# stanfordnlp/mac-network

Hardware: AMD Instinct MI355X
Metric: questions/sec fwd+bwd (B=64,d=512,p=12,KB=14x14x1024) at 1/2/4/8 MI355X (higher is better)
Workload: dtype f32 (3xfp16-split emulation); 1 GPU

## Files before the change

include/macx.h:

```cpp
#ifndef MACX_H
#define MACX_H

#include <stddef.h>
#include <stdint.h>

#ifdef __cplusplus
extern "C" {
#endif

#define MACX_ABI_VERSION 5

enum {
  MACX_OK = 0,
  MACX_EINVAL = -1,
  MACX_EUNSUPPORTED = -2,
  MACX_EREJECTED = -3,
  MACX_ESMALL = -4,
  MACX_EWAIT = -5
};

enum { MACX_ACT_NON = 0, MACX_ACT_TANH = 1, MACX_ACT_SIGMOID = 2, MACX_ACT_ELU = 3, MACX_ACT_RELU = 4 };
enum { MACX_INIT_PRM = 0, MACX_INIT_ZERO = 1, MACX_INIT_Q = 2 };
enum { MACX_WRITE_MEM = 0, MACX_WRITE_INFO = 1, MACX_WRITE_SUM = 2, MACX_WRITE_BOTH = 3 };

typedef struct macx_opts {
  int32_t abi_version;
  int32_t init_ctrl, init_mem;
  int32_t control_input_unshared;
  int32_t control_input_act;
  int32_t control_feed_prev;
  int32_t control_feed_prev_att;
  int32_t control_feed_inputs;
  int32_t control_cont_act;
  int32_t read_mem_act;
  int32_t read_ctrl_act;
  int32_t write_inputs;
  int32_t write_self_att;
  int32_t write_self_att_cont;
  int32_t write_mem_act;
  int32_t write_gate;
  int32_t write_gate_shared;
  float   write_gate_bias;
  int32_t memory_variational_dropout;
  int32_t gemm_family;
  int32_t tune[16];
} macx_opts;
#define MACX_TUNE(v) ((v) + 1)
enum {
  MACX_TUNE_NATIVE_WAVES = 0,
  MACX_TUNE_PHASE_MASK = 1,
  MACX_TUNE_ROW_TILES = 2,
  MACX_TUNE_CHAIN = 4,
  MACX_TUNE_SB_DEFER = 5,
  MACX_TUNE_CHAIN_KV = 7,
  MACX_TUNE_SB_WIDE = 8,
  MACX_TUNE_WGRAD_PIPE = 10,
  MACX_TUNE_SB_CONT = 13,
  MACX_TUNE_DKB_UNI = 14,
  MACX_TUNE_PRE_FILL = 3,
  MACX_TUNE_DKB_FILL = 15
};

typedef struct macx_shapes {
  int32_t B;
  int32_t S;
  int32_t N;
  int32_t d;
  int32_t p;
  int32_t b0;
  int32_t d_logical;
} macx_shapes;

typedef struct macx_dropout {
  float keep_memory, keep_read, keep_write;
  uint32_t seed;
  const uint32_t* mask_word;
} macx_dropout;

typedef struct macx_params {
  const float* initMem;
  const float* initCtrl;
  const float* qInput_W;
  const float* qInput_b;
  const float* qInputU_W;
  const float* qInputU_b;
  const float* ctrlLogits_w;
  const float* ctrlLogits_b;
  const float* contControl_W;
  const float* contControl_b;
  const float* contControl2_W;
  const float* contControl2_b;
  const float* projX_W;
  const float* projX_b;
  const float* projY_W;
  const float* projY_b;
  const float* memKbProj_W;
  const float* memKbProj_b;
  const float* memKbProj2_W;
  const float* memKbProj2_b;
  const float* kbLogits_w;
  const float* kbLogits_b;
  const float* newMemory_W;
  const float* newMemory_b;
  const float* selfCtrl_W;
  const float* selfCtrl_b;
  const float* selfLogits_w;
  const float* selfLogits_b;
  const float* gate_W;
  const float* gate_b;
} macx_params;

typedef struct macx_param_grads {
  float* initMem; float* initCtrl;
  float* qInput_W; float* qInput_b; float* qInputU_W; float* qInputU_b;
  float* ctrlLogits_w; float* ctrlLogits_b;
  float* contControl_W; float* contControl_b; float* contControl2_W; float* contControl2_b;
  float* projX_W; float* projX_b; float* projY_W; float* projY_b;
  float* memKbProj_W; float* memKbProj_b; float* memKbProj2_W; float* memKbProj2_b;
  float* kbLogits_w; float* kbLogits_b;
  float* newMemory_W; float* newMemory_b;
  float* selfCtrl_W; float* selfCtrl_b; float* selfLogits_w; float* selfLogits_b;
  float* gate_W; float* gate_b;
} macx_param_grads;

typedef struct macx_inputs {
  const float* vecQuestions;
  const float* words;
  const int32_t* questionLengths;
  const float* knowledgeBase;
} macx_inputs;

typedef struct macx_input_grads {
  float* vecQuestions;
  float* words;
  float* knowledgeBase;
} macx_input_grads;

enum {
  MACX_SEG_CONTROLS = 0,
// ... 207 lines not shown
```

mac-network_amd/_lib.py:

```python
import ctypes as C
import os

from . import build as _build

ABI_VERSION = 5

MACX_OK, MACX_EINVAL, MACX_EUNSUPPORTED, MACX_EREJECTED, MACX_ESMALL, MACX_EWAIT = 0, -1, -2, -3, -4, -5
HANDOFF_BITS = {1: "a chain tile gave up waiting for its step's y", 2: "a filler workgroup gave up waiting for the previous step's write unit"}
STATUS_WORDS = 16
ACT = {"NON": 0, "TANH": 1, "SIGMOID": 2, "ELU": 3, "RELU": 4}
INIT = {"PRM": 0, "ZERO": 1, "Q": 2}
WRITE_INPUTS = {"MEM": 0, "INFO": 1, "SUM": 2, "BOTH": 3}
SEG = {"controls": 0, "memories": 1, "infos": 2, "att_question": 3, "att_kb": 4, "att_self": 5, "att_gate": 6,
       "status": 7}


class MacxOpts(C.Structure):
    _fields_ = [(n, C.c_int32) for n in (
        "abi_version", "init_ctrl", "init_mem", "control_input_unshared", "control_input_act", "control_feed_prev",
        "control_feed_prev_att", "control_feed_inputs", "control_cont_act", "read_mem_act", "read_ctrl_act",
        "write_inputs", "write_self_att", "write_self_att_cont", "write_mem_act", "write_gate", "write_gate_shared")]
    _fields_ += [("write_gate_bias", C.c_float), ("memory_variational_dropout", C.c_int32), ("gemm_family", C.c_int32),
                 ("tune", C.c_int32 * 16)]


TUNE = {"native_waves": 0, "phase_mask": 1, "row_tiles": 2, "pre_fill": 3, "chain": 4, "sb_defer": 5, "chain_kv": 7, "sb_wide": 8,
        "wgrad_pipe": 10, "sb_cont": 13, "dkb_uni": 14, "dkb_fill": 15}


def set_tune(opts, key, value):
    k = TUNE[key] if isinstance(key, str) else int(key)
    if k not in TUNE.values():
        raise KeyError("no tuning key %r (have %s)" % (key, sorted(TUNE)))
    opts.tune[k] = 0 if value is None else int(value) + 1


class MacxShapes(C.Structure):
    _fields_ = [(n, C.c_int32) for n in ("B", "S", "N", "d", "p", "b0", "d_logical")]


class MacxDropout(C.Structure):
    _fields_ = [("keep_memory", C.c_float), ("keep_read", C.c_float), ("keep_write", C.c_float), ("seed", C.c_uint32),
                ("mask_word", C.c_void_p)]


PARAM_FIELDS = (
    "initMem", "initCtrl", "qInput_W", "qInput_b", "qInputU_W", "qInputU_b", "ctrlLogits_w", "ctrlLogits_b",
    "contControl_W", "contControl_b", "contControl2_W", "contControl2_b", "projX_W", "projX_b", "projY_W", "projY_b",
    "memKbProj_W", "memKbProj_b", "memKbProj2_W", "memKbProj2_b", "kbLogits_w", "kbLogits_b", "newMemory_W",
    "newMemory_b", "selfCtrl_W", "selfCtrl_b", "selfLogits_w", "selfLogits_b", "gate_W", "gate_b")


class MacxParams(C.Structure):
    _fields_ = [(n, C.c_void_p) for n in PARAM_FIELDS]


class MacxParamGrads(C.Structure):
    _fields_ = [(n, C.c_void_p) for n in PARAM_FIELDS]


class MacxOutShapes(C.Structure):
    _fields_ = [(n, C.c_int32) for n in ("B", "d", "hidden", "answers", "b0")]


OUT_FIELDS = ("outQuestion_W", "outQuestion_b", "fc0_W", "fc0_b", "fc1_W", "fc1_b")


class MacxOutParams(C.Structure):
    _fields_ = [(n, C.c_void_p) for n in OUT_FIELDS]


class MacxOutGrads(C.Structure):
    _fields_ = [(n, C.c_void_p) for n in OUT_FIELDS]


class MacxStemShapes(C.Structure):
    _fields_ = [(n, C.c_int32) for n in ("B", "H", "W", "Cin", "Cmid", "Cout", "b0")]


STEM_FIELDS = ("kernel0", "bias0", "kernel1", "bias1")


class MacxStemParams(C.Structure):
    _fields_ = [(n, C.c_void_p) for n in STEM_FIELDS]


class MacxStemGrads(C.Structure):
    _fields_ = [(n, C.c_void_p) for n in STEM_FIELDS]


class MacxConvShapes(C.Structure):
    _fields_ = [(n, C.c_int32) for n in ("B", "H", "W", "Cin", "Cout", "k", "stride")]


class MacxEncShapes(C.Structure):
    _fields_ = [(n, C.c_int32) for n in ("B", "S", "V", "E", "h", "b0")]


ENC_FIELDS = ("emb", "fw_kernel", "fw_bias", "bw_kernel", "bw_bias")


class MacxEncParams(C.Structure):
    _fields_ = [(n, C.c_void_p) for n in ENC_FIELDS]


class MacxEncGrads(C.Structure):
    _fields_ = [(n, C.c_void_p) for n in ENC_FIELDS]


# ... 191 lines not shown
```

mac-network_amd/csrc/macx_api.hip:

```cpp
#include <hip/hip_runtime.h>
#include <math.h>
#include <stdlib.h>
#include <string.h>

#include "../../include/macx.h"
#include "macx_common.hip.h"
#include "macx_gemm.hip.h"
#include "macx_gemm6.hip.h"
#include "macx_gemm_tn.hip.h"
#include "macx_wgrad6.hip.h"
#include "macx_gemm3h.hip.h"
#include "macx_h2.hip.h"
#include "macx_gemm_h2.hip.h"
#include "macx_chain_api.hip.h"
#include "macx_wgrad_h2.hip.h"
#include "macx_small.hip.h"
#include "macx_ops.hip.h"
#include "macx_conv.hip.h"

using namespace macx;

#define CK(expr)                         \
  do {                                   \
    hipError_t _e = (expr);              \
// ... 1642 lines not shown
}

int CellBwd::initial_state_bwd() {
  if (o->init_mem == MACX_INIT_PRM) CK(rs.add(DM, B, d, d, GP->initMem, st));
  else if (o->init_mem == MACX_INIT_Q && o->init_ctrl == MACX_INIT_Q) CK(axpy(DM, Bd, GI->vecQuestions, st));
  if (o->init_ctrl == MACX_INIT_PRM) CK(rs.add(DC, B, d, d, GP->initCtrl, st));
  return MACX_OK;
}

int CellBwd::read_linear_wgrads() {
  CKI(wb.add(saved + L.md, d, ws + W.DY, d, p * B, d, d, GP->projY_W, st));
  CK(rs.add(ws + W.DY, p * B, d, d, GP->projY_b, st));
  return MACX_OK;
}

int CellBwd::write_linear_wgrads() {
  const int rows = p * B;
  CKI(wb.add(memories(), d, dwlin_all, d, rows, d, d, GP->newMemory_W, st));
  CKI(wb.add(saved + L.seg[MACX_SEG_INFOS], d, dwlin_all, d, rows, d, d, GP->newMemory_W + dd, st));
  if (o->write_self_att)
    CKI(wb.add(saved + L.self_smry, d, dwlin_all, d, rows, d, d, GP->newMemory_W + 2 * dd, st));
  CK(rs.add(dwlin_all, rows, d, d, GP->newMemory_b, st));
  return MACX_OK;
}

int CellBwd::read_weight_contractions() {
  int ns_w = (int)W.ns_big;
  if (h2) {
    int* ecom = reinterpret_cast<int*>(ws + W.ecom);
    constexpr int ES = EMIN_NB * 8;
    {
      EminList el;
      memset(&el, 0, sizeof(el));
      el.R = B * N; el.C = d; el.part = ecom;
      el.base[0] = reinterpret_cast<const char*>(saved + L.H1); el.stride[0] = L.act_stride * sizeof(float); el.nt[0] = p;
      el.base[1] = reinterpret_cast<const char*>(ws + W.dI2); el.stride[1] = W.act_floats * sizeof(float); el.nt[1] = p;
      el.base[2] = reinterpret_cast<const char*>(saved + L.KBd); el.stride[2] = L.act_stride * sizeof(float); el.nt[2] = rdrop ? p : 1;
      el.base[3] = reinterpret_cast<const char*>(ws + W.dX); el.stride[3] = W.act_floats * sizeof(float); el.nt[3] = p;
      CK(emin_list(el, 4, st));
    }
    TnH2P t;
    memset(&t, 0, sizeof(t));
    ns_w = (wgrad_pipe_mode() >= 3 && wgrad_h2_kw(d) == 2 && wgrad_h2_jw(d) == 2 && W.ns_big >= 2) ? (int)W.ns_big / 2 : (int)W.ns_big;
    t.M = p * B * N; t.Kd = d; t.Jd = d; t.nsplit = ns_w; t.rows_per_split = rows_per_split(t.M, t.nsplit);
    t.R = B * N;
    t.A = reinterpret_cast<const char*>(saved + L.H1); t.a_stride = L.act_stride * sizeof(float); t.a_mod = 0;
    t.G = reinterpret_cast<const char*>(ws + W.dI2); t.g_stride = W.act_floats * sizeof(float);
    t.ecomA = ecom; t.ecomG = ecom + ES; t.ecom_nb = EMIN_NB;
    t.ftab = reinterpret_cast<uint16_t*>(ws + W.wg_ftab);
    t.dbg = kb_gemm_dbg();
    t.part = ws + W.slab_w2;
    const TnH2P t_w2 = t;
    t.A = reinterpret_cast<const char*>(saved + L.KBd);
    t.a_mod = rdrop ? 0 : B * N;
    t.G = reinterpret_cast<const char*>(ws + W.dX);
    t.ecomA = ecom + 2 * ES; t.ecomG = ecom + 3 * ES;
    t.part = ws + W.slab_wx;
    t.ftab = reinterpret_cast<uint16_t*>(ws + W.wg_ftab2);
    CK(wgrad_h2_launch_pair(t_w2, t, st));
  } else {
    TnP t;
    memset(&t, 0, sizeof(t));
    t.M = p * B * N; t.Kd = d; t.Jd = d; t.nsplit = (int)W.ns_big; t.rows_per_split = rows_per_split(t.M, t.nsplit);
    t.A = saved + L.H1; t.lda = d; t.a_mod = t.M; t.G = ws + W.dI2; t.ldg = d;
    t.part = ws + W.slab_w2;
    CK(wgrad_any(t, st));
    if (rdrop) { t.A = saved + L.KBd; t.a_mod = t.M; }
    else { t.A = in->knowledgeBase; t.a_mod = B * N; }
    t.G = ws + W.dX;
    t.part = ws + W.slab_wx;
    CK(wgrad_any(t, st));
  }
  if (h2 && W.sb_deferred) {
    SbH2P q;
    memset(&q, 0, sizeof(q));
    q.B = B; q.N = N; q.d = d; q.qpg = sb_qpg(B, N);
    q.X = h2_view(saved + L.X, B * N, d); q.dI1 = h2_view(ws + W.dI1, B * N, d);
    q.y = saved + L.y; q.W1a = P->memKbProj_W;
    q.dW1a_part = ws + W.slab_w1a; q.dW1b_part = ws + W.slab_w1b; q.dy_part = nullptr;
    q.nsteps = p;
    q.x_step = L.act_stride * sizeof(float); q.g_step = W.dI1_stride * sizeof(float); q.y_step = Bd;
    q.dbg = kb_gemm_dbg();
    q.qpg = W.sb_qpg;
    CK(W.sb_wide ? sb_h2w_launch(q, st) : sb_h2_launch(q, st));
  }
  const int nslab1 = (int)((h2 && W.sb_deferred ? 1 : p) * W.ngroup);
  SlabList sl;
  sl.d[0] = SlabDesc{ws + W.slab_w2, ns_w, dd / 4, GP->memKbProj2_W, 0};
  sl.d[1] = SlabDesc{ws + W.slab_wx, ns_w, dd / 4, GP->projX_W, 0};
  sl.d[2] = SlabDesc{ws + W.slab_w1a, nslab1, dd / 4, GP->memKbProj_W, 0};
  sl.d[3] = SlabDesc{ws + W.slab_w1b, nslab1, dd / 4, GP->memKbProj_W + dd, 0};
  CK(slab_reduce_list_launch(sl, 4, dd, st));
  CK(rs.add(ws + W.db2_part, p * (int)W.dwk_rows, d, d, GP->memKbProj2_b, st));
  CK(rs.add(ws + W.db1_part, p * (int)W.db_rows, d, d, GP->memKbProj_b, st));
  CK(rs.add(ws + W.dbx_part, p * (int)W.db_rows, d, d, GP->projX_b, st));
  CK(rs.add(ws + W.dwk_part, p * (int)W.dwk_rows, d, d, GP->kbLogits_w, st));
  CK(rs.add(ws + W.dbk_part, p * B, 1, 1, GP->kbLogits_b, st));
  CK(rs.run(st));
  return MACX_OK;
}
}

int macx_cell_backward_phase(const macx_opts* o, const macx_shapes* s, const macx_dropout* dp, const macx_params* P,
                             const macx_inputs* in, const float* saved, size_t saved_floats, float* ws, size_t ws_floats,
                             const float* d_memory, const float* d_control, const macx_param_grads* GP,
                             const macx_input_grads* GI, int phase, void* stream) {
  ModeScope ms(o);
  if (phase < 0 || phase > 2) return MACX_EINVAL;
  CKI(check_impl(o, s));
  if (!dp || !P || !in || !saved || !ws || !GP || !GI) return MACX_EINVAL;
  if (!GI->knowledgeBase || !GI->words || !GI->vecQuestions) return MACX_EINVAL;
  CellBwd r(o, s, dp, P, in, saved, ws, GP, GI, stream);
  CKI(r.check_bwd_buffers(saved_floats, ws_floats, phase));
  if (phase != 2) {
    CKI(r.init_state_grads(d_memory, d_control));
    if (o->control_feed_prev) {
      CK(dev_zero(GI->words, (size_t)r.B * s->S * r.d * sizeof(float), r.st));
      CK(dev_zero(ws + r.W.dwc_part, r.Bd * sizeof(float), r.st));
      CK(dev_zero(ws + r.W.dccx, (size_t)(r.p + 1) * r.Bd * sizeof(float), r.st));
      r.dc_in_loop = true;
    }
    r.plan_dkb_fill();
    for (int i = r.p - 1; i >= 0; --i) {
      CKI(r.write_unit_bwd(i));
      CKI(r.read_unit_bwd(i));
      CKI(r.dy_linear_bwd(i, true));
      if (o->control_feed_prev) CKI(r.control_step_bwd(i));
    }
    CKI(r.read_dc_reduce_all());
    CKI(r.control_bwd_tail());
    CKI(r.gate_wgrads());
    CKI(r.control_inputs_bwd());
    CKI(r.initial_state_bwd());
    CKI(r.read_linear_wgrads());
    CKI(r.write_linear_wgrads());
    CKI(r.wb.run(r.st));
  }
  CK(r.rs.run(r.st));
  return phase == 1 ? MACX_OK : r.read_weight_contractions();
}

int macx_cell_backward(const macx_opts* o, const macx_shapes* s, const macx_dropout* dp, const macx_params* P,
                       const macx_inputs* in, const float* saved, size_t saved_floats, float* ws, size_t ws_floats,
                       const float* d_memory, const float* d_control, const macx_param_grads* GP,
                       const macx_input_grads* GI, void* stream) {
  return macx_cell_backward_phase(o, s, dp, P, in, saved, saved_floats, ws, ws_floats, d_memory, d_control, GP, GI, 0, stream);
}

namespace {
int unit_check(const macx_opts* o, const macx_shapes* s, bool write) {
  CKI(check_impl(o, s));
  if (s->p != 1) return MACX_EINVAL;
  if (write && o->write_self_att) return MACX_EUNSUPPORTED;
  return MACX_OK;
}
}

size_t macx_workspace_bytes(const macx_opts* o, const macx_shapes* s, int for_backward) {
  return macx_ws_floats(o, s, for_backward) * sizeof(float);
}

int macx_read_fwd(const macx_opts* o, const macx_shapes* s, const macx_dropout* dp, const macx_params* P,
                  const float* knowledgeBase, const float* memory, const float* control, float* saved, size_t saved_floats,
                  float* info, float* att, void* stream) {
  ModeScope ms(o);
  CKI(unit_check(o, s, false));
// ... 1137 lines not shown
```

mac-network_amd/csrc/macx_wgrad_h2.hip.h:

```cpp
#pragma once
#include "macx_gemm_tn.hip.h"
#include "macx_h2.hip.h"

namespace macx {

__device__ __forceinline__ float sum16_h2(float v) {
  v += __shfl_xor(v, 1, 64);
  v += __shfl_xor(v, 2, 64);
  v += __shfl_xor(v, 4, 64);
  v += __shfl_xor(v, 8, 64);
  return v;
}
__device__ __forceinline__ uint32_t pk_mul_f16(uint32_t a, uint32_t b) {
  return __builtin_bit_cast(uint32_t, __builtin_bit_cast(f16x2_t, a) * __builtin_bit_cast(f16x2_t, b));
}
__device__ __forceinline__ uint32_t pk_pow2_f16(int k) {
  const float f = k < -30 ? 0.f : h2_pow2(k);
  return pk_f16(f, f);
}

struct ReadAttBwdH2P {
  int B, N, d;
  const float* att;
  const float* da;
// ... 412 lines not shown
          wh_mfma<NR, NC>(af, gf[0], acc);
        }
        if (p.dbg & 2048) wait_vmcnt<0>(); else wait_vmcnt_n(my_n);
        __syncthreads();
      }
      wait_vmcnt<0>();
    }
  } else
  if (nchunk > 0) {
    const int my_n = (NI + (wave == 0 ? 1 : 0)) * (RING - 2);
#pragma unroll
    for (int s = 0; s < RING - 1; ++s) issue(s);
    wait_vmcnt_n(my_n);
    __syncthreads();
#pragma unroll 1
    for (int s = 0; s < nchunk; ++s) {
      if (!(p.dbg & 2048)) issue(s + RING - 1);
      if (!(p.dbg & 1024)) wh_compute<NR, NC>(tiles_a(s % RING), APL, tiles_g(s % RING), GPL, factors(s % RING), lane, acc);
      wait_vmcnt_n(my_n);
      __syncthreads();
    }
    wait_vmcnt<0>();
  }

  __syncthreads();

  const float sc = h2_unscale(h2_emin_final(p.ecomA, p.ecom_nb, tk * KW + aq), h2_emin_final(p.ecomG, p.ecom_nb, tj * JW + gq));
  float* out = p.part + (size_t)split * p.Kd * p.Jd + (size_t)(tk * KT + wr * 16 * NR) * p.Jd + tj * JT + wc * 32 * JW;
  float* tw = reinterpret_cast<float*>(lds) + wave * (32 * wh_slab_ldw<NC>());
#pragma unroll
  for (int tp = 0; tp < NR; tp += 2) wh_store_slab<2>(acc, tp, sc, tw, out, p.Jd, lane);
}

inline int wgrad_h2_jw(int Jd) { return (Jd % 256 == 0) ? 2 : 1; }
inline int wgrad_h2_kw(int Kd) { return (Kd % 256 == 0) ? 2 : 1; }
inline int wgrad_h2_tiles(int Kd, int Jd) { return (Kd / (wgrad_h2_kw(Kd) * T_TILE)) * (Jd / (wgrad_h2_jw(Jd) * T_TILE)); }

inline hipError_t wgrad_h2_factors_launch(const TnH2P& a, const TnH2P& b, int ny, hipStream_t st) {
  if (a.rows_per_split % 32 != 0 || !a.ftab || !b.ftab) return hipErrorInvalidValue;
  const size_t mpad = wgrad_h2_mpad((size_t)a.M);
  hipLaunchKernelGGL(wgrad_h2_factors_kernel, dim3((unsigned)((mpad + 255) / 256), ny), dim3(256), 0, st, a, b);
  return hipGetLastError();
}
template <int KW, int JW, int PIPE = 0>
inline hipError_t wgrad_h2_launch_t(const TnH2P& a, const TnH2P& b, int ny, hipStream_t st) {
  auto kern = wgrad_h2_kernel<KW, JW, PIPE>;
  constexpr size_t lds = (size_t)wh_ring<KW, JW>() * wh_stage_bytes<KW, JW>();
  hipError_t e = lds_attr_once(reinterpret_cast<const void*>(kern), lds);
  if (e != hipSuccess) return e;
  hipLaunchKernelGGL(kern, dim3(wgrad_h2_tiles(a.Kd, a.Jd) * a.nsplit, ny), dim3(512), lds, st, a, b);
  return hipGetLastError();
}
inline hipError_t wgrad_h2_launch(const TnH2P& p, hipStream_t st) {
  hipError_t e = wgrad_h2_factors_launch(p, p, 1, st);
  if (e != hipSuccess) return e;
  const int kw = wgrad_h2_kw(p.Kd), jw = wgrad_h2_jw(p.Jd);
  if (kw == 2 && jw == 2) return wgrad_pipe_mode() ? wgrad_h2_launch_t<2, 2, 1>(p, p, 1, st) : wgrad_h2_launch_t<2, 2, 0>(p, p, 1, st);
  if (kw == 2) return wgrad_h2_launch_t<2, 1>(p, p, 1, st);
  return jw == 2 ? wgrad_h2_launch_t<1, 2>(p, p, 1, st) : wgrad_h2_launch_t<1, 1>(p, p, 1, st);
}
inline hipError_t wgrad_h2_launch_pair(const TnH2P& a, const TnH2P& b, hipStream_t st) {
  const bool same = a.M == b.M && a.Kd == b.Kd && a.Jd == b.Jd && a.nsplit == b.nsplit && a.rows_per_split == b.rows_per_split && a.R == b.R;
  if (!(same && wgrad_pipe_mode() >= 2 && wgrad_h2_kw(a.Kd) == 2 && wgrad_h2_jw(a.Jd) == 2 && a.ftab != b.ftab && a.part != b.part)) {
    hipError_t e = wgrad_h2_launch(a, st);
    return e != hipSuccess ? e : wgrad_h2_launch(b, st);
  }
  hipError_t e = wgrad_h2_factors_launch(a, b, 2, st);
  return e != hipSuccess ? e : wgrad_h2_launch_t<2, 2, 1>(a, b, 2, st);
}

struct SbH2P {
  int B, N, d;
  int qpg;
  H2View X;
  H2View dI1;
  const float* y;
  const float* W1a;
  float* dW1a_part;
  float* dW1b_part;
  float* dy_part;
  int nsteps;
  size_t x_step, g_step, y_step;
  int dbg;
};

constexpr int SBH_STAGE = 4 * WH_APL;
constexpr int SBH_CW = 8;
constexpr int SBH_MAXROWS = 4096;
constexpr int SBH_RING = 4;
constexpr int SBH_MAXQ = 32;

template <bool DY>
__global__ __launch_bounds__(512) void sb_h2_kernel(SbH2P p) {
  extern __shared__ __attribute__((aligned(16))) float smem[];
  char* lds = reinterpret_cast<char*>(smem);
  uint16_t* ftab = reinterpret_cast<uint16_t*>(lds + SBH_RING * SBH_STAGE);
  float* ytab = reinterpret_cast<float*>(lds + SBH_RING * SBH_STAGE + SBH_MAXROWS * 2);
  float* sctab = ytab + SBH_MAXQ * T_TILE;
  int* qmn = reinterpret_cast<int*>(sctab + SBH_MAXQ);

  const int nt = p.d / T_TILE;
  const int ntile = nt * nt;
  const int nblk = gridDim.x;
  int v = blockIdx.x;
  if ((nblk & 7) == 0) v = (blockIdx.x & 7) * (nblk >> 3) + (blockIdx.x >> 3);
  const int group = v / ntile;
  const int tile = v % ntile;
  const int tk = tile / nt, tj = tile % nt;

  const int tid = threadIdx.x, lane = tid & 63;
  const int wave = __builtin_amdgcn_readfirstlane(tid >> 6);
  const int wr = wave >> 2, wc = wave & 3;

  const int nchunk = (p.N + 31) >> 5;
  const int b_begin = group * p.qpg;
  const int b_end = min(p.B, b_begin + p.qpg);
  const int nq = b_end - b_begin;
  const int total = nq * nchunk;
  const size_t Rp = p.X.Rp();
  const size_t xpb = p.X.plane_bytes(), gpb = p.dI1.plane_bytes();
  const int xcb = p.X.cb(), gcb = p.dI1.cb();
  H2View vX = p.X, vG = p.dI1;
  const float* yS = p.y;
  const int rows_q = nchunk * 32;

  const WhSlot sl = wh_slot(lane);
  auto issue = [&](int s_raw) __attribute__((always_inline)) {
    const int s = min(s_raw, total - 1);
    const int qi = s / nchunk, ch = s - qi * nchunk;
    const int n = sl.row(ch * 32, p.N);
    const size_t row = (size_t)(b_begin + qi) * p.N + n;
    char* st = lds + (s_raw % SBH_RING) * SBH_STAGE;
#pragma unroll
    for (int j = 0; j < 4; ++j) {
      const int u = wave * 4 + j;
      const int im = u >> 3, ct = u & 7;
      const char* src = (im < 2 ? vX.base + (im & 1) * xpb + ((size_t)(tk * 16 + 2 * ct + sl.kg) * Rp + row) * 16
                                : vG.base + (im & 1) * gpb + ((size_t)(tj * 16 + 2 * ct + sl.kg) * Rp + row) * 16);
      dma16b(src, st + im * WH_APL + ct * 1024);
    }
  };
  auto tables = [&]() __attribute__((always_inline)) {
  if (tid < 2 * SBH_MAXQ) qmn[tid] = 127;
  __syncthreads();
  for (int i0 = 0; i0 < nq * rows_q; i0 += 512) {
    const int i = i0 + tid;
    const int qi = i / rows_q, n = i - qi * rows_q;
    int ex = 127, eg = 127;
    if (i < nq * rows_q && n < p.N) {
      const size_t row = (size_t)(b_begin + qi) * p.N + n;
      ex = (int)vX.exps()[row * xcb + tk];
      eg = (int)vG.exps()[row * gcb + tj];
    }
    const int q_lo = min(i0 + (tid & ~63), nq * rows_q - 1) / rows_q, q_hi = min(i0 + (tid | 63), nq * rows_q - 1) / rows_q;
    for (int q = q_lo; q <= q_hi; ++q) {
      int mx = qi == q ? ex : 127, mg = qi == q ? eg : 127;
#pragma unroll
      for (int o = 32; o > 0; o >>= 1) { mx = min(mx, __shfl_xor(mx, o, 64)); mg = min(mg, __shfl_xor(mg, o, 64)); }
      if (lane == 0) { atomicMin(qmn + q, mx); atomicMin(qmn + SBH_MAXQ + q, mg); }
    }
  }
  __syncthreads();
  for (int i = tid; i < nq * rows_q; i += 512) {
    const int qi = i / rows_q, n = i - qi * rows_q;
    const int b = b_begin + qi;
    uint16_t f = 0;
// ... 38 lines not shown
  auto consume = [&](int b) __attribute__((always_inline)) {
    const float sc = sctab[b - b_begin];
    f32x4 y4[4];
#pragma unroll
    for (int t = 0; t < 4; ++t) y4[t] = *reinterpret_cast<const f32x4*>(ytab + (b - b_begin) * T_TILE + wr * 64 + t * 16 + (lane >> 4) * 4);
#pragma unroll
    for (int t = 0; t < 4; ++t)
#pragma unroll
      for (int e = 0; e < 4; ++e) {
        const int k = tk * T_TILE + wr * 64 + t * 16 + (lane >> 4) * 4 + e;
        const float yk = y4[t][e];
        float dyp = 0.f;
#pragma unroll
        for (int c = 0; c < 2; ++c) {
          const float sv = accS[t][c][e] * sc;
          accB[t][c][e] += sv;
          accA[t][c][e] = fmaf(yk, sv, accA[t][c][e]);
          if (DY) dyp = fmaf(w1[t][e][c], sv, dyp);
          accS[t][c][e] = 0.f;
        }
        if (DY) {
          dyp = sum16_h2(dyp);
          if ((lane & 15) == 0) p.dy_part[((size_t)(tj * 4 + wc) * p.B + b) * p.d + k] = dyp;
        }
      }
  };

#pragma unroll 1
  for (int step = 0; step < p.nsteps; ++step) {
  vX.base = p.X.base + (size_t)step * p.x_step; vG.base = p.dI1.base + (size_t)step * p.g_step;
  yS = p.y + (size_t)step * p.y_step;
  if (total > 0) {
    issue(0);
    issue(1);
    issue(2);
  }
  tables();
  if (total > 0) {
    wait_vmcnt<8>();
    __syncthreads();
    int qi = 0, qch = 0;
#pragma unroll 1
    for (int s = 0; s < total; ++s) {
      if (!(p.dbg & 2048)) issue(s + 3);
      if (!(p.dbg & 1024)) compute(s % SBH_RING, qi, qch);
      wait_vmcnt<8>();
      if (++qch == nchunk) {
        if (!(p.dbg & 512)) consume(b_begin + qi);
        qch = 0; ++qi;
      }
      __syncthreads();
    }
    wait_vmcnt<0>();
  }
  __syncthreads();
  }

  float* oa = p.dW1a_part + (size_t)group * p.d * p.d;
  float* ob = p.dW1b_part + (size_t)group * p.d * p.d;
  constexpr int LDW = 36;
  float* tw = reinterpret_cast<float*>(lds) + wave * (64 * LDW);
#pragma unroll
  for (int which = 0; which < 2; ++which) {
#pragma unroll
    for (int t = 0; t < 4; ++t)
#pragma unroll
      for (int c = 0; c < 2; ++c)
#pragma unroll
        for (int e = 0; e < 4; ++e)
          tw[(t * 16 + (lane >> 4) * 4 + e) * LDW + c * 16 + (lane & 15)] = which ? accB[t][c][e] : accA[t][c][e];
    float* o = (which ? ob : oa) + (size_t)(tk * T_TILE + wr * 64) * p.d + tj * T_TILE + wc * 32;
#pragma unroll
    for (int i = 0; i < 8; ++i) {
      const int r = i * 8 + (lane >> 3), c4 = (lane & 7) * 4;
      *reinterpret_cast<f32x4*>(o + (size_t)r * p.d + c4) = *reinterpret_cast<const f32x4*>(tw + r * LDW + c4);
    }
  }
}

constexpr int SBW_STAGE = 2 * WH_APL + 4 * WH_APL;
constexpr int SBW_RING = 3;
constexpr int SBW_MAXQ = 4;
constexpr int SBW_MAXROWS = 1024;

constexpr int SBW_TABLES = SBW_MAXROWS * 2 + SBW_MAXQ * T_TILE * 4 + 4 * SBW_MAXQ * 4;
template <bool CONT>
__global__ __launch_bounds__(512) void sb_h2w_kernel(SbH2P p) {
  extern __shared__ __attribute__((aligned(16))) float smem[];
  char* lds = reinterpret_cast<char*>(smem);
  char* tab0 = lds + SBW_RING * SBW_STAGE;
  uint16_t* ftab = reinterpret_cast<uint16_t*>(tab0);
  float* ytab = reinterpret_cast<float*>(tab0 + SBW_MAXROWS * 2);
  int* qmn = reinterpret_cast<int*>(ytab + SBW_MAXQ * T_TILE);
  float* yold = reinterpret_cast<float*>(tab0 + (CONT ? 2 : 1) * SBW_TABLES);

  const int ntk = p.d / T_TILE, ntj = p.d / (2 * T_TILE);
  const int ntile = ntk * ntj;
  const int nblk = gridDim.x;
  int v = blockIdx.x;
  if ((nblk & 7) == 0) v = (blockIdx.x & 7) * (nblk >> 3) + (blockIdx.x >> 3);
  const int group = v / ntile;
  const int tile = v % ntile;
  const int tk = tile / ntj, tj = tile % ntj;

  const int tid = threadIdx.x, lane = tid & 63;
  const int wave = __builtin_amdgcn_readfirstlane(tid >> 6);
  const int wr = wave >> 2, wc = wave & 3;
  const int gq = wc >> 1;

  const int nchunk = (p.N + 31) >> 5;
  const int b_begin = group * p.qpg;
  const int b_end = min(p.B, b_begin + p.qpg);
  const int nq = b_end - b_begin;
  const int total = nq * nchunk;
  const size_t Rp = p.X.Rp();
  const size_t xpb = p.X.plane_bytes(), gpb = p.dI1.plane_bytes();
  const int xcb = p.X.cb(), gcb = p.dI1.cb();
  H2View vX = p.X, vG = p.dI1;
  const float* yS = p.y;
  const int rows_q = nchunk * 32;

  const WhSlot sl = wh_slot(lane);
  const uint32_t lds0 = lds_addr_of(lds);
  auto issue = [&](int s_raw, int s, const char* xb, const char* gb) __attribute__((always_inline)) {
    const int qi = s / nchunk, ch = s - qi * nchunk;
    const int n = sl.row(ch * 32, p.N);
    const uint32_t voff = (uint32_t)(((size_t)sl.kg * Rp + (size_t)(b_begin + qi) * p.N + n) * 16);
    const uint32_t st = lds0 + (uint32_t)((s_raw % SBW_RING) * SBW_STAGE);
#pragma unroll
    for (int j = 0; j < 2; ++j) {
      const int u = wave * 2 + j, pl = u >> 3, ct = u & 7;
      dma16b_s(xb + pl * xpb + (size_t)(tk * 16 + 2 * ct) * Rp * 16, voff, st + pl * WH_APL + ct * 1024);
    }
#pragma unroll
    for (int j = 0; j < 4; ++j) {
      const int u = wave * 4 + j, pl = u >> 4, ct = u & 15;
      dma16b_s(gb + pl * gpb + (size_t)(tj * 32 + 2 * ct) * Rp * 16, voff, st + 2 * WH_APL + pl * 2 * WH_APL + ct * 1024);
    }
  };
  uint16_t* ftab_c = ftab;
  float* ytab_c = ytab;
  int* qmn_c = qmn;
  auto tables = [&]() __attribute__((always_inline)) {
    if (tid < 3 * SBW_MAXQ) qmn[tid] = 127;
    __syncthreads();
    for (int i0 = 0; i0 < nq * rows_q; i0 += 512) {
      const int i = i0 + tid;
      const int qi = i / rows_q, n = i - qi * rows_q;
      int ex = 127, eg0 = 127, eg1 = 127;
      if (i < nq * rows_q && n < p.N) {
        const size_t row = (size_t)(b_begin + qi) * p.N + n;
        ex = (int)vX.exps()[row * xcb + tk];
        eg0 = (int)vG.exps()[row * gcb + 2 * tj];
        eg1 = (int)vG.exps()[row * gcb + 2 * tj + 1];
      }
      const int q_lo = min(i0 + (tid & ~63), nq * rows_q - 1) / rows_q, q_hi = min(i0 + (tid | 63), nq * rows_q - 1) / rows_q;
      for (int q = q_lo; q <= q_hi; ++q) {
        int mx = qi == q ? ex : 127, mg = qi == q ? min(eg0, eg1) : 127;
#pragma unroll
        for (int o = 32; o > 0; o >>= 1) { mx = min(mx, __shfl_xor(mx, o, 64)); mg = min(mg, __shfl_xor(mg, o, 64)); }
        if (lane == 0) { atomicMin(qmn + q, mx); atomicMin(qmn + SBW_MAXQ + q, mg); }
      }
    }
    __syncthreads();
    for (int i = tid; i < 2 * nq * rows_q; i += 512) {
      const int blk = i / (nq * rows_q), r = i - blk * nq * rows_q;
      const int qi = r / rows_q, n = r - qi * rows_q;
      uint16_t f = 0;
      if (n < p.N) {
        const size_t row = (size_t)(b_begin + qi) * p.N + n;
        const int k = (min(qmn[qi], 126) - (int)vX.exps()[row * xcb + tk]) + (min(qmn[SBW_MAXQ + qi], 126) - (int)vG.exps()[row * gcb + 2 * tj + blk]);
        f = (uint16_t)(pk_pow2_f16(k) & 0xFFFFu);
      }
      ftab[blk * (SBW_MAXROWS / 2) + r] = f;
    }
    for (int i = tid; i < nq * T_TILE; i += 512)
      ytab[i] = yS[(size_t)(b_begin + (i >> 7)) * p.d + tk * T_TILE + (i & 127)];
  };

  f32x4 accT[4][4], accA[4][4];
#pragma unroll
  for (int t = 0; t < 4; ++t)
#pragma unroll
    for (int c = 0; c < 4; ++c) accT[t][c] = accA[t][c] = f32x4{0.f, 0.f, 0.f, 0.f};

  auto compute = [&](int buf, int qi, int ch) __attribute__((always_inline)) {
    const char* st = lds + buf * SBW_STAGE;
    wh_compute<4, 4>(st + (wr * 4) * 1024, WH_APL, st + 2 * WH_APL + (wc * 4) * 1024, 2 * WH_APL,
                     ftab_c + gq * (SBW_MAXROWS / 2) + qi * rows_q + ch * 32, lane, accT);
  };
  int ex_prev = 0, eg_prev = 0, ybuf = 0;
  bool pending = false;
  auto keep_y = [&](const float* ynext) __attribute__((always_inline)) {
    if (tid < T_TILE) yold[(ybuf ^ 1) * T_TILE + tid] = ynext ? ynext[tid] : 0.f;
    ybuf ^= 1;
  };
  auto fold = [&](const float* ynext, int ex_next, int eg_next) __attribute__((always_inline)) {
    const float sc = h2_unscale(ex_prev, eg_prev);
    const float mv = h2_pow2(max(min((ex_next + eg_next) - (ex_prev + eg_prev), 126), -126));
    const float* yp = yold + ybuf * T_TILE;
#pragma unroll
    for (int t = 0; t < 4; ++t) {
      const int k0 = wr * 64 + t * 16 + (lane >> 4) * 4;
      f32x4 yn = f32x4{0.f, 0.f, 0.f, 0.f};
      if (ynext) yn = *reinterpret_cast<const f32x4*>(ynext + k0);
      const f32x4 yo = *reinterpret_cast<const f32x4*>(yp + k0);
#pragma unroll
      for (int e = 0; e < 4; ++e) {
        const float dy = (yo[e] - yn[e]) * sc;
#pragma unroll
        for (int c = 0; c < 4; ++c) {
          accA[t][c][e] = fmaf(dy, accT[t][c][e], accA[t][c][e]);
          accT[t][c][e] *= mv;
        }
      }
    }
    keep_y(ynext);
    ex_prev = ex_next; eg_prev = eg_next;
  };

  if constexpr (CONT) {
    const int G = p.nsteps * total;
    auto issue_g = [&](int g_raw) __attribute__((always_inline)) {
      const int g = min(g_raw, G - 1);
      const int ist = g / total;
      issue(g_raw, g - ist * total, p.X.base + (size_t)ist * p.x_step, p.dI1.base + (size_t)ist * p.g_step);
    };
    issue_g(0);
    issue_g(1);
    tables();
    wait_vmcnt<6>();
    __syncthreads();
    const int nrows = nq * rows_q;
    const int t_q = min(tid, nrows - 1) / rows_q, t_n = min(tid, nrows - 1) - t_q * rows_q;
    const bool t_row = tid < nrows && t_n < p.N;
    const size_t t_grow = (size_t)(b_begin + t_q) * p.N + min(t_n, p.N - 1);
    const bool t_yv = tid < nq * T_TILE;
    const size_t t_yoff = (size_t)(b_begin + (t_yv ? (tid >> 7) : 0)) * p.d + tk * T_TILE + (tid & 127);
    int t_ex = 127, t_g0 = 127, t_g1 = 127;
    float t_y = 0.f;
    int step = 0, sg = 0, qi = 0, qch = 0;
#pragma unroll 1
    for (int g = 0; g < G; ++g) {
      const bool more = step + 1 < p.nsteps;
      char* nset = tab0 + ((step + 1) & 1) * SBW_TABLES;
      uint16_t* ftab_n = reinterpret_cast<uint16_t*>(nset);
      float* ytab_n = reinterpret_cast<float*>(nset + SBW_MAXROWS * 2);
      int* qmn_n = reinterpret_cast<int*>(ytab_n + SBW_MAXQ * T_TILE);
      if (more && sg == 1) {
        const H2View nX{const_cast<char*>(p.X.base) + (size_t)(step + 1) * p.x_step, p.X.R, p.X.C};
        const H2View nG{const_cast<char*>(p.dI1.base) + (size_t)(step + 1) * p.g_step, p.dI1.R, p.dI1.C};
        const int8_t* ax = nX.exps() + t_grow * xcb + tk;
        const int8_t* ag = nG.exps() + t_grow * gcb + 2 * tj;
        const float* ay = p.y + (size_t)(step + 1) * p.y_step + t_yoff;
        asm volatile("global_load_sbyte %0, %1, off" : "=v"(t_ex) : "v"(ax) : "memory");
        asm volatile("global_load_sbyte %0, %1, off" : "=v"(t_g0) : "v"(ag) : "memory");
        asm volatile("global_load_sbyte %0, %1, off offset:1" : "=v"(t_g1) : "v"(ag) : "memory");
        asm volatile("global_load_dword %0, %1, off" : "=v"(t_y) : "v"(ay) : "memory");
      }
      if (!(p.dbg & 2048)) issue_g(g + 2);
      if (qch == 0) {
        const float* yn = ytab_c + qi * T_TILE;
        const int exn = min(qmn_c[qi], 126), egn = min(qmn_c[SBW_MAXQ + qi], 126);
        if (pending) {
          if (!(p.dbg & 512)) fold(yn, exn, egn);
        } else {
          keep_y(yn);
          ex_prev = exn; eg_prev = egn;
          pending = true;
        }
      }
      if (!(p.dbg & 1024)) compute(g % SBW_RING, qi, qch);
      if (p.dbg & 2048) wait_vmcnt<0>(); else wait_vmcnt<6>();
      if (more) {
        if (sg == 0) {
          if (tid < 3 * SBW_MAXQ) qmn_n[tid] = 127;
        } else if (sg == 1) {
          asm volatile("" : "+v"(t_ex), "+v"(t_g0), "+v"(t_g1), "+v"(t_y));
          if (!t_row) { t_ex = 127; t_g0 = 127; t_g1 = 127; }
          const int q_lo = min(tid & ~63, nrows - 1) / rows_q, q_hi = min(tid | 63, nrows - 1) / rows_q;
          for (int q = q_lo; q <= q_hi; ++q) {
            int mx = t_q == q ? t_ex : 127, mg = t_q == q ? min(t_g0, t_g1) : 127;
#pragma unroll
            for (int o = 32; o > 0; o >>= 1) { mx = min(mx, __shfl_xor(mx, o, 64)); mg = min(mg, __shfl_xor(mg, o, 64)); }
            if (lane == 0) { atomicMin(qmn_n + q, mx); atomicMin(qmn_n + SBW_MAXQ + q, mg); }
          }
        } else if (sg == 2) {
          if (tid < nrows) {
            const int bx = min(qmn_n[t_q], 126), bg = min(qmn_n[SBW_MAXQ + t_q], 126);
            ftab_n[tid] = t_row ? (uint16_t)(pk_pow2_f16((bx - t_ex) + (bg - t_g0)) & 0xFFFFu) : (uint16_t)0;
            ftab_n[(SBW_MAXROWS / 2) + tid] = t_row ? (uint16_t)(pk_pow2_f16((bx - t_ex) + (bg - t_g1)) & 0xFFFFu) : (uint16_t)0;
          }
          if (t_yv) ytab_n[tid] = t_y;
        }
      }
      if (++qch == nchunk) { qch = 0; ++qi; }
      if (++sg == total) {
        sg = 0; qi = 0; ++step;
        char* cset = tab0 + (step & 1) * SBW_TABLES;
        ftab_c = reinterpret_cast<uint16_t*>(cset);
        ytab_c = reinterpret_cast<float*>(cset + SBW_MAXROWS * 2);
        qmn_c = reinterpret_cast<int*>(ytab_c + SBW_MAXQ * T_TILE);
      }
      __syncthreads();
    }
    wait_vmcnt<0>();
    __syncthreads();
  } else {
#pragma unroll 1
  for (int step = 0; step < p.nsteps; ++step) {
    vX.base = p.X.base + (size_t)step * p.x_step; vG.base = p.dI1.base + (size_t)step * p.g_step;
    yS = p.y + (size_t)step * p.y_step;
    auto issue_s = [&](int s_raw) __attribute__((always_inline)) { issue(s_raw, min(s_raw, total - 1), vX.base, vG.base); };
    if (total > 0) { issue_s(0); issue_s(1); }
    tables();
    if (total > 0) {
      wait_vmcnt<6>();
      __syncthreads();
      int qi = 0, qch = 0;
#pragma unroll 1
      for (int s = 0; s < total; ++s) {
        if (!(p.dbg & 2048)) issue_s(s + 2);
        if (qch == 0) {
          const float* yn = ytab + qi * T_TILE;
          const int exn = min(qmn[qi], 126), egn = min(qmn[SBW_MAXQ + qi], 126);
          if (pending) {
            if (!(p.dbg & 512)) fold(yn, exn, egn);
          } else {
            keep_y(yn);
            ex_prev = exn; eg_prev = egn;
            pending = true;
          }
        }
        if (!(p.dbg & 1024)) compute(s % SBW_RING, qi, qch);
        wait_vmcnt<6>();
        if (++qch == nchunk) { qch = 0; ++qi; }
        __syncthreads();
      }
      wait_vmcnt<0>();
    }
    __syncthreads();
  }
  }
  if (pending && !(p.dbg & 512)) fold(nullptr, ex_prev, eg_prev);
  const float scT = h2_unscale(ex_prev, eg_prev);

  float* tw = reinterpret_cast<float*>(lds) + wave * (64 * wh_slab_ldw<4>());
  const size_t o = (size_t)group * p.d * p.d + (size_t)(tk * T_TILE + wr * 64) * p.d + tj * 2 * T_TILE + wc * 64;
  wh_store_slab<4>(accA, 0, 1.f, tw, p.dW1a_part + o, p.d, lane);
  wh_store_slab<4>(accT, 0, scT, tw, p.dW1b_part + o, p.d, lane);
}

inline bool sb_h2_wide_ok(int B, int N, int d) { return d % 256 == 0 && B >= 1 && N >= 1 && ((N + 31) / 32) * 32 <= SBW_MAXROWS / 2; }
inline int sb_h2_wide_qpg(int B, int N, int d) {
  const int tiles = (d / 128) * (d / 256);
  int groups = 256 / tiles;
  if (groups < 1) groups = 1;
  int qpg = (B + groups - 1) / groups;
  const int rows_q = ((N + 31) / 32) * 32;
  const int cap = min(SBW_MAXQ, (SBW_MAXROWS / 2) / rows_q);
  if (qpg > cap) qpg = cap;
  return qpg < 1 ? 1 : qpg;
}
inline int sb_cont_mode() { return tune_get(MACX_TUNE_SB_CONT, 1); }
inline hipError_t sb_h2w_launch(const SbH2P& p, hipStream_t st) {
  const int nchunk = (p.N + 31) >> 5;
  if (p.qpg < 1 || p.qpg > SBW_MAXQ || p.qpg * nchunk * 32 > SBW_MAXROWS / 2 || p.d % 256 || p.dy_part || p.nsteps < 1) return hipErrorInvalidValue;
  const int ngroup = (p.B + p.qpg - 1) / p.qpg;
  const bool cont = sb_cont_mode() && p.nsteps > 1 && nchunk >= 3 && p.qpg * nchunk * 32 <= 512;
  if (cont) {
    constexpr size_t lds = (size_t)SBW_RING * SBW_STAGE + 2 * SBW_TABLES + 2 * T_TILE * 4;
    static_assert(lds <= 160 * 1024, "two table sets fit beside the ring");
    hipError_t e = lds_attr_once(reinterpret_cast<const void*>(sb_h2w_kernel<true>), lds);
    if (e != hipSuccess) return e;
    hipLaunchKernelGGL(sb_h2w_kernel<true>, dim3((p.d / 128) * (p.d / 256) * ngroup), dim3(512), lds, st, p);
    return hipGetLastError();
  }
  constexpr size_t lds = (size_t)SBW_RING * SBW_STAGE + SBW_TABLES + 2 * T_TILE * 4;
  hipError_t e = lds_attr_once(reinterpret_cast<const void*>(sb_h2w_kernel<false>), lds);
  if (e != hipSuccess) return e;
  hipLaunchKernelGGL(sb_h2w_kernel<false>, dim3((p.d / 128) * (p.d / 256) * ngroup), dim3(512), lds, st, p);
  return hipGetLastError();
}

inline hipError_t sb_h2_launch(const SbH2P& p, hipStream_t st) {
  const int nchunk = (p.N + 31) >> 5;
  if (p.qpg * nchunk * 32 > SBH_MAXROWS || p.qpg > SBH_MAXQ) return hipErrorInvalidValue;
  constexpr size_t lds = SBH_RING * SBH_STAGE + SBH_MAXROWS * 2 + SBH_MAXQ * T_TILE * 4 + SBH_MAXQ * 4 + 2 * SBH_MAXQ * 4;
  if (p.nsteps < 1 || (p.nsteps > 1 && p.dy_part)) return hipErrorInvalidValue;
  auto kern = p.dy_part ? sb_h2_kernel<true> : sb_h2_kernel<false>;
  hipError_t e = lds_attr_once(reinterpret_cast<const void*>(kern), lds);
  if (e != hipSuccess) return e;
  const int nt = p.d / T_TILE;
  const int ngroup = (p.B + p.qpg - 1) / p.qpg;
  hipLaunchKernelGGL(kern, dim3(nt * nt * ngroup), dim3(512), lds, st, p);
  return hipGetLastError();
}

}
```

Baseline: 16940 questions/s.

## Replace per-stage workgroup barrier with LDS counter hand-off in deferred dW1 kernel

In the continuous-stream variant of the wide deferred dW1a/dW1b kernel, the per-stage __syncthreads is replaced by a ring of LDS counters that waves increment with ds_add and spin on with a sleep. Each wave signals after finishing its table phase and the first MFMA of a stage, and waits only for the slot it needs before reusing a ring stage. The intent is to let waves drift relative to one another and overlap MFMA work with loads, instead of stalling the whole workgroup every stage. It adds spin-wait overhead and a bounded timeout that poisons the outputs with NaN and sets a status bit if a wave gives up, which risks ordering bugs if the counter protocol is wrong.

Result: no change. 16960 questions/s (median of 2 runs) (+0.1%).

```diff
diff --git a/include/macx.h b/include/macx.h
--- a/include/macx.h
+++ b/include/macx.h
@@ -55,6 +55,7 @@
   MACX_TUNE_CHAIN_KV = 7,
   MACX_TUNE_SB_WIDE = 8,
   MACX_TUNE_WGRAD_PIPE = 10,
+  MACX_TUNE_SB_HANDOFF = 6,
   MACX_TUNE_SB_CONT = 13,
   MACX_TUNE_DKB_UNI = 14,
   MACX_TUNE_PRE_FILL = 3,
diff --git a/mac-network_amd/_lib.py b/mac-network_amd/_lib.py
--- a/mac-network_amd/_lib.py
+++ b/mac-network_amd/_lib.py
@@ -6,7 +6,8 @@
 ABI_VERSION = 5
 
 MACX_OK, MACX_EINVAL, MACX_EUNSUPPORTED, MACX_EREJECTED, MACX_ESMALL, MACX_EWAIT = 0, -1, -2, -3, -4, -5
-HANDOFF_BITS = {1: "a chain tile gave up waiting for its step's y", 2: "a filler workgroup gave up waiting for the previous step's write unit"}
+HANDOFF_BITS = {1: "a chain tile gave up waiting for its step's y", 2: "a filler workgroup gave up waiting for the previous step's write unit",
+                4: "a wave of the deferred dW1a / dW1b launch gave up waiting for the other waves of its workgroup"}
 STATUS_WORDS = 16
 ACT = {"NON": 0, "TANH": 1, "SIGMOID": 2, "ELU": 3, "RELU": 4}
 INIT = {"PRM": 0, "ZERO": 1, "Q": 2}
@@ -24,7 +25,7 @@
                  ("tune", C.c_int32 * 16)]
 
 
-TUNE = {"native_waves": 0, "phase_mask": 1, "row_tiles": 2, "pre_fill": 3, "chain": 4, "sb_defer": 5, "chain_kv": 7, "sb_wide": 8,
+TUNE = {"native_waves": 0, "phase_mask": 1, "row_tiles": 2, "pre_fill": 3, "chain": 4, "sb_defer": 5, "sb_handoff": 6, "chain_kv": 7, "sb_wide": 8,
         "wgrad_pipe": 10, "sb_cont": 13, "dkb_uni": 14, "dkb_fill": 15}
 
 
diff --git a/mac-network_amd/csrc/macx_api.hip b/mac-network_amd/csrc/macx_api.hip
--- a/mac-network_amd/csrc/macx_api.hip
+++ b/mac-network_amd/csrc/macx_api.hip
@@ -1748,6 +1748,7 @@
     q.x_step = L.act_stride * sizeof(float); q.g_step = W.dI1_stride * sizeof(float); q.y_step = Bd;
     q.dbg = kb_gemm_dbg();
     q.qpg = W.sb_qpg;
+    q.status = reinterpret_cast<uint32_t*>(saved + L.status);
     CK(W.sb_wide ? sb_h2w_launch(q, st) : sb_h2_launch(q, st));
   }
   const int nslab1 = (int)((h2 && W.sb_deferred ? 1 : p) * W.ngroup);
diff --git a/mac-network_amd/csrc/macx_wgrad_h2.hip.h b/mac-network_amd/csrc/macx_wgrad_h2.hip.h
--- a/mac-network_amd/csrc/macx_wgrad_h2.hip.h
+++ b/mac-network_amd/csrc/macx_wgrad_h2.hip.h
@@ -518,6 +518,7 @@
   int nsteps;
   size_t x_step, g_step, y_step;
   int dbg;
+  uint32_t* status;
 };
 
 constexpr int SBH_STAGE = 4 * WH_APL;
@@ -722,10 +723,33 @@
 constexpr int SBW_RING = 3;
 constexpr int SBW_MAXQ = 4;
 constexpr int SBW_MAXROWS = 1024;
+constexpr int SB_HANDOFF_DEFAULT = 1;
 
 constexpr int SBW_TABLES = SBW_MAXROWS * 2 + SBW_MAXQ * T_TILE * 4 + 4 * SBW_MAXQ * 4;
-template <bool CONT>
+
+constexpr uint32_t SBW_WAIT_BUDGET = 1u << 20;
+constexpr uint32_t HANDOFF_SBW = 4;
+__device__ __forceinline__ uint32_t sbw_peek(uint32_t lds_addr) {
+  uint32_t v;
+  asm volatile("ds_read_b32 %0, %1\n\ts_waitcnt lgkmcnt(0)" : "=v"(v) : "v"(lds_addr) : "memory");
+  return __builtin_amdgcn_readfirstlane(v);
+}
+__device__ __forceinline__ void sbw_signal(uint32_t lds_addr, int lane) {
+  asm volatile("s_waitcnt lgkmcnt(0)" ::: "memory");
+  if (lane == 0) asm volatile("ds_add_u32 %0, %1" ::"v"(lds_addr), "v"(1u) : "memory");
+}
+__device__ __forceinline__ bool sbw_wait(uint32_t lds_addr, uint32_t want) {
+  uint32_t spins = 0;
+  while (sbw_peek(lds_addr) < want) {
+    if (spins++ >= SBW_WAIT_BUDGET) return false;
+    __builtin_amdgcn_s_sleep(1);
+  }
+  return true;
+}
+
+template <bool CONT, bool HANDOFF = false>
 __global__ __launch_bounds__(512) void sb_h2w_kernel(SbH2P p) {
+  static_assert(CONT || !HANDOFF, "the hand-off belongs to the stage stream");
   extern __shared__ __attribute__((aligned(16))) float smem[];
   char* lds = reinterpret_cast<char*>(smem);
   char* tab0 = lds + SBW_RING * SBW_STAGE;
@@ -733,6 +757,7 @@
   float* ytab = reinterpret_cast<float*>(tab0 + SBW_MAXROWS * 2);
   int* qmn = reinterpret_cast<int*>(ytab + SBW_MAXQ * T_TILE);
   float* yold = reinterpret_cast<float*>(tab0 + (CONT ? 2 : 1) * SBW_TABLES);
+  uint32_t* hs = reinterpret_cast<uint32_t*>(yold + 2 * T_TILE);
 
   const int ntk = p.d / T_TILE, ntj = p.d / (2 * T_TILE);
   const int ntile = ntk * ntj;
@@ -869,8 +894,12 @@
     issue_g(0);
     issue_g(1);
     tables();
+    if (HANDOFF && tid < 4) hs[tid] = tid == 0 ? 8u : 0u;
     wait_vmcnt<6>();
     __syncthreads();
+    const uint32_t hs0 = lds_addr_of(hs);
+    uint32_t slot = 0, lap8 = 8;
+    bool gave_up = false;
     const int nrows = nq * rows_q;
     const int t_q = min(tid, nrows - 1) / rows_q, t_n = min(tid, nrows - 1) - t_q * rows_q;
     const bool t_row = tid < nrows && t_n < p.N;
@@ -898,6 +927,9 @@
         asm volatile("global_load_sbyte %0, %1, off offset:1" : "=v"(t_g1) : "v"(ag) : "memory");
         asm volatile("global_load_dword %0, %1, off" : "=v"(t_y) : "v"(ay) : "memory");
       }
+      if constexpr (HANDOFF) {
+        if (!gave_up && !sbw_wait(hs0 + 4 * slot, lap8)) gave_up = true;
+      }
       if (!(p.dbg & 2048)) issue_g(g + 2);
       if (qch == 0) {
         const float* yn = ytab_c + qi * T_TILE;
@@ -910,9 +942,8 @@
           pending = true;
         }
       }
-      if (!(p.dbg & 1024)) compute(g % SBW_RING, qi, qch);
-      if (p.dbg & 2048) wait_vmcnt<0>(); else wait_vmcnt<6>();
-      if (more) {
+      auto table_phase = [&]() __attribute__((always_inline)) {
+        if (!more) return;
         if (sg == 0) {
           if (tid < 3 * SBW_MAXQ) qmn_n[tid] = 127;
         } else if (sg == 1) {
@@ -933,6 +964,29 @@
           }
           if (t_yv) ytab_n[tid] = t_y;
         }
+      };
+      if constexpr (HANDOFF) {
+        const char* st = lds + (g % SBW_RING) * SBW_STAGE;
+        const char* sa = st + (wr * 4) * 1024;
+        u32x4 gf[2][4], al[4], ah[4];
+        if (!(p.dbg & 1024)) {
+          wh_load_g<4>(st + 2 * WH_APL + (wc * 4) * 1024, 2 * WH_APL, ftab_c + gq * (SBW_MAXROWS / 2) + qi * rows_q + qch * 32, lane, gf);
+          wh_load_a<4>(sa + WH_APL, lane, al);
+          wh_load_a<4>(sa, lane, ah);
+          wh_mfma<4, 4>(al, gf[0], accT);
+        }
+        if (p.dbg & 2048) wait_vmcnt<0>(); else wait_vmcnt<6>();
+        table_phase();
+        if (++slot == SBW_RING) { slot = 0; lap8 += 8; }
+        sbw_signal(hs0 + 4 * slot, lane);
+        if (!(p.dbg & 1024)) {
+          wh_mfma<4, 4>(ah, gf[1], accT);
+          wh_mfma<4, 4>(ah, gf[0], accT);
+        }
+      } else {
+        if (!(p.dbg & 1024)) compute(g % SBW_RING, qi, qch);
+        if (p.dbg & 2048) wait_vmcnt<0>(); else wait_vmcnt<6>();
+        table_phase();
       }
       if (++qch == nchunk) { qch = 0; ++qi; }
       if (++sg == total) {
@@ -942,10 +996,25 @@
         ytab_c = reinterpret_cast<float*>(cset + SBW_MAXROWS * 2);
         qmn_c = reinterpret_cast<int*>(ytab_c + SBW_MAXQ * T_TILE);
       }
-      __syncthreads();
+      if constexpr (!HANDOFF) __syncthreads();
     }
     wait_vmcnt<0>();
+    if (HANDOFF && gave_up && lane == 0) hs[3] = 1u;
     __syncthreads();
+    if constexpr (HANDOFF) {
+      if (hs[3]) {
+        const float nan = __uint_as_float(0x7fc00000u);
+#pragma unroll
+        for (int t = 0; t < 4; ++t)
+#pragma unroll
+          for (int c = 0; c < 4; ++c) accT[t][c] = accA[t][c] = f32x4{nan, nan, nan, nan};
+        if (tid == 0 && p.status) {
+          __hip_atomic_fetch_or(p.status, HANDOFF_SBW, __ATOMIC_RELAXED, __HIP_MEMORY_SCOPE_AGENT);
+          uint32_t none = 0u;
+          __hip_atomic_compare_exchange_strong(p.status + 1, &none, 1u, __ATOMIC_RELAXED, __ATOMIC_RELAXED, __HIP_MEMORY_SCOPE_AGENT);
+        }
+      }
+    }
   } else {
 #pragma unroll 1
   for (int step = 0; step < p.nsteps; ++step) {
@@ -1003,17 +1072,19 @@
   return qpg < 1 ? 1 : qpg;
 }
 inline int sb_cont_mode() { return tune_get(MACX_TUNE_SB_CONT, 1); }
+inline int sb_handoff_mode() { return tune_get(MACX_TUNE_SB_HANDOFF, SB_HANDOFF_DEFAULT); }
 inline hipError_t sb_h2w_launch(const SbH2P& p, hipStream_t st) {
   const int nchunk = (p.N + 31) >> 5;
   if (p.qpg < 1 || p.qpg > SBW_MAXQ || p.qpg * nchunk * 32 > SBW_MAXROWS / 2 || p.d % 256 || p.dy_part || p.nsteps < 1) return hipErrorInvalidValue;
   const int ngroup = (p.B + p.qpg - 1) / p.qpg;
   const bool cont = sb_cont_mode() && p.nsteps > 1 && nchunk >= 3 && p.qpg * nchunk * 32 <= 512;
   if (cont) {
-    constexpr size_t lds = (size_t)SBW_RING * SBW_STAGE + 2 * SBW_TABLES + 2 * T_TILE * 4;
+    constexpr size_t lds = (size_t)SBW_RING * SBW_STAGE + 2 * SBW_TABLES + 2 * T_TILE * 4 + 16;
     static_assert(lds <= 160 * 1024, "two table sets fit beside the ring");
-    hipError_t e = lds_attr_once(reinterpret_cast<const void*>(sb_h2w_kernel<true>), lds);
+    auto kern = sb_handoff_mode() ? sb_h2w_kernel<true, true> : sb_h2w_kernel<true, false>;
+    hipError_t e = lds_attr_once(reinterpret_cast<const void*>(kern), lds);
     if (e != hipSuccess) return e;
-    hipLaunchKernelGGL(sb_h2w_kernel<true>, dim3((p.d / 128) * (p.d / 256) * ngroup), dim3(512), lds, st, p);
+    hipLaunchKernelGGL(kern, dim3((p.d / 128) * (p.d / 256) * ngroup), dim3(512), lds, st, p);
     return hipGetLastError();
   }
   constexpr size_t lds = (size_t)SBW_RING * SBW_STAGE + SBW_TABLES + 2 * T_TILE * 4;
```
